# adamjorr/kbbq-py

Measured on AMD Instinct MI355X. Metric: bases/sec recalibrated (2x150 bp), higher is better.
Workload: dtype u8

## Files before the change

### kbbq-py_amd/csrc/kbbq_hip.hip

```cpp
#include "kbbq_kernels.h"
#include "kbbq_kernels_v3.h"
#include "kbbq_k2_tile.h"
#include "kbbq_solve_kernels.h"
#include "kbbq_lut_kernels.h"
#include "kbbq_aligned_kernels.h"
#include "kbbq_layout_kernels.h"
#include "kbbq_apply_aligned.h"
#include "kbbq_kmer.h"
#include "../../include/kbbq_hip.h"
#include "host_threads.h"

#include <algorithm>
#include <climits>
#include <cstdint>
#include <cstdarg>
#include <cstdio>
#include <cstring>
#include <functional>
#include <string>
#include <thread>
#include <vector>

static thread_local std::string g_err;

static int fail(int code, const char* fmt, ...)
{
    char buf[512];
    va_list ap; va_start(ap, fmt); vsnprintf(buf, sizeof buf, fmt, ap); va_end(ap);
    g_err = buf;
    return code;
}

static bool env_is(const char* name, const char* value) { const char* v = getenv(name); return v && !strcmp(v, value); }

int kbbq_set_error_(int code, const char* msg) { g_err = msg ? msg : ""; return code; }

#define HIPCHK(expr)                                                                   \
    do {                                                                               \
        hipError_t e_ = (expr);                                                        \
        if (e_ != hipSuccess)                                                          \
            return fail(KBBQ_E_HIP, "%s failed: %s (%s:%d)", #expr, hipGetErrorString(e_), \
                        __FILE__, __LINE__);                                           \
    } while (0)

struct DevScratch { void* p = nullptr; size_t bytes = 0; };

struct kbbq_ctx {
    int device = 0;
    int cus = 0;
    int lds_bytes = 0;
    char name[128] = {0};
    hipStream_t own_stream = nullptr;
    hipStream_t stream = nullptr;
    u64* d_status = nullptr;
    int* d_stats = nullptr;
    DevScratch wgplan;
    DevScratch ops4;
    DevScratch tally;
    DevScratch rowlut;
    void* stage_host[2] = {nullptr, nullptr}; void* stage_dev[2] = {nullptr, nullptr}; size_t stage_bytes = 0;
    hipStream_t stage_stream = nullptr;
    hipStream_t stage_down_stream = nullptr;
    hipEvent_t stage_up[2] = {nullptr, nullptr}, stage_used[2] = {nullptr, nullptr}, stage_down[2] = {nullptr, nullptr};
    bool timing = false;
    std::vector<std::pair<hipEvent_t, hipEvent_t>> ev[2];
    double ms_acc[2] = {0.0, 0.0};
    int64_t launches[2] = {0, 0};
};

#define KBBQ_NSTATUS 8

constexpr size_t K2T_ROW_LUT_MAX = 52 << 10;
constexpr int K2V3_FRONTS = 8;
constexpr int K2T_XCD_TILES = 1;
constexpr int K2T_XCD = 8;
constexpr int K7_FRONTS = 8;
constexpr int TALLY_K4_SHARE = 8;
static const u64 ST_INIT[KBBQ_NSTATUS] = {~0ull, ~0ull, ~0ull, ~0ull, ~0ull, ~0ull, ~0ull, ~0ull};

enum K1Form { K1_ROWS, K1_ALIGNED, K1_ALIGNED_REF, K1_BANDS };
struct K1Variant { K1Form form; int dn, nib, kj; const void* kernel[2]; };
#define K1_SPLITS(K, ...) {(const void*)(K<false, __VA_ARGS__>), (const void*)(K<true, __VA_ARGS__>)}
static const K1Variant K1_VARIANTS[] = {
    {K1_ROWS, K1V3_DNREP, 0, 0, K1_SPLITS(k1v3_accumulate, K1V3_DNREP)},
    {K1_ROWS, 8, 0, 0, K1_SPLITS(k1v3_accumulate, 8)},
    {K1_ROWS, K1V3_DNREP, 1, 0, K1_SPLITS(k1v3_accumulate, K1V3_DNREP, true)},
    {K1_ROWS, 8, 1, 0, K1_SPLITS(k1v3_accumulate, 8, true)},
    {K1_ROWS, K1V3_DNREP, 1, 13, K1_SPLITS(k1v3_accumulate, K1V3_DNREP, true, 13)},
    {K1_ROWS, K1V3_DNREP, 1, 19, K1_SPLITS(k1v3_accumulate, K1V3_DNREP, true, 19)},
    {K1_ALIGNED, K1V3_DNREP, 0, 0, K1_SPLITS(k1v3_aligned, K1V3_DNREP)},
    {K1_ALIGNED, 8, 0, 0, K1_SPLITS(k1v3_aligned, 8)},
    {K1_ALIGNED_REF, K1V3_DNREP, 0, 0, K1_SPLITS(k1v3_aligned_ref, K1V3_DNREP)},
    {K1_ALIGNED_REF, 8, 0, 0, K1_SPLITS(k1v3_aligned_ref, 8)},
    {K1_BANDS, 0, 0, 0, K1_SPLITS(k1v3_bands, false)},
    {K1_BANDS, 0, 1, 0, K1_SPLITS(k1v3_bands, true)},
};
#undef K1_SPLITS

static const void* k1_kernel(K1Form form, bool split, int dn, int nib, int kj)
{
    for (const K1Variant& v : K1_VARIANTS)
        if (v.form == form && v.dn == dn && v.nib == nib && v.kj == kj) return v.kernel[split];
    return nullptr;
}

enum LdsKernel { LK_K1_PLAIN, LK_K1_PLAIN_SPLIT, LK_K2V3, LK_K2V3_NIB, LK_K2T, LK_K2T_NIB, LK_K2T_BANDS, LK_K2_LDS16, LK_K2_LDS8, LK_COUNT };
static const void* const LDS_KERNELS[LK_COUNT] = {
    (const void*)k1_accumulate<false>, (const void*)k1_accumulate<true>,
    (const void*)k2v3_apply<false>, (const void*)k2v3_apply<true>,
    (const void*)k2t_apply<false>, (const void*)k2t_apply<true>, (const void*)k2t_bands,
    (const void*)k2_apply<int16_t, true, true>, (const void*)k2_apply<int8_t, true, false>,
};

extern "C" {

int kbbq_abi_version(void) { return KBBQ_ABI_VERSION; }
const char* kbbq_last_error(void) { return g_err.c_str(); }

int kbbq_device_count(int* count)
{
    int n = 0;
    hipError_t e = hipGetDeviceCount(&n);
    if (e != hipSuccess) { *count = 0; return fail(KBBQ_E_HIP, "hipGetDeviceCount: %s", hipGetErrorString(e)); }
    *count = n;
    return KBBQ_OK;
}

int kbbq_bind_host_to_device(int device, int* numa_node, int* ncpus)
{
    char busid[64] = {0};
    HIPCHK(hipDeviceGetPCIBusId(busid, (int)sizeof busid, device));
    return kbbq_bind_host_to_pci(busid, numa_node, ncpus);
}

int kbbq_ctx_create(int device, kbbq_ctx** out)
{
    if (!out) return fail(KBBQ_E_ARG, "kbbq_ctx_create: out is NULL");
    *out = nullptr;
    const bool dbg = getenv("KBBQ_CTX_DBG") != nullptr;
    auto t_prev = std::chrono::steady_clock::now();
    auto lap = [&](const char* what) {
        if (!dbg) return;
        const auto t = std::chrono::steady_clock::now();
        fprintf(stderr, "[kbbq_ctx_create] %-28s %7.2f ms\n", what, std::chrono::duration<double, std::milli>(t - t_prev).count());
        t_prev = t;
    };
    HIPCHK(hipSetDevice(device));
    lap("hipSetDevice");
    hipDeviceProp_t prop;
    HIPCHK(hipGetDeviceProperties(&prop, device));
    lap("hipGetDeviceProperties");
    if (strncmp(prop.gcnArchName, "gfx950", 6) != 0)
        return fail(KBBQ_E_HIP, "libkbbq_hip is built for gfx950 only; device %d is %s", device, prop.gcnArchName);
    kbbq_ctx* c = new kbbq_ctx();
    c->device = device;
    c->cus = prop.multiProcessorCount;
    c->lds_bytes = (int)prop.maxSharedMemoryPerMultiProcessor;
    if (c->lds_bytes <= 0) c->lds_bytes = 160 * 1024;
    snprintf(c->name, sizeof c->name, "%s (%s)", prop.name, prop.gcnArchName);
    hipError_t e = hipStreamCreateWithFlags(&c->own_stream, hipStreamNonBlocking);
    if (e != hipSuccess) { delete c; return fail(KBBQ_E_HIP, "hipStreamCreate: %s", hipGetErrorString(e)); }
    c->stream = c->own_stream;
    lap("hipStreamCreate");
    e = hipMalloc((void**)&c->d_status, sizeof ST_INIT);
    if (e != hipSuccess) { (void)hipStreamDestroy(c->own_stream); delete c; return fail(KBBQ_E_HIP, "hipMalloc(status): %s", hipGetErrorString(e)); }
    e = hipMemcpy(c->d_status, ST_INIT, sizeof ST_INIT, hipMemcpyHostToDevice);
    if (e != hipSuccess) { (void)hipFree(c->d_status); (void)hipStreamDestroy(c->own_stream); delete c; return fail(KBBQ_E_HIP, "hipMemcpy(status): %s", hipGetErrorString(e)); }
    lap("hipMalloc + hipMemcpy");
    auto full_lds = [&](const void* kernel) {
        (void)hipFuncSetAttribute(kernel, hipFuncAttributeMaxDynamicSharedMemorySize, c->lds_bytes);
        if (kernel == LDS_KERNELS[0]) lap("first hipFuncSetAttribute");
    };
    for (const void* kernel : LDS_KERNELS) full_lds(kernel);
    for (const K1Variant& v : K1_VARIANTS) { full_lds(v.kernel[0]); full_lds(v.kernel[1]); }
    (void)hipGetLastError();
    lap("the other attributes");
    *out = c;
    return KBBQ_OK;
}

int kbbq_ctx_destroy(kbbq_ctx* c)
{
    if (!c) return KBBQ_OK;
    (void)hipSetDevice(c->device);
    for (int w = 0; w < 2; ++w)
        for (auto& pr : c->ev[w]) { (void)hipEventDestroy(pr.first); (void)hipEventDestroy(pr.second); }
    if (c->d_status) (void)hipFree(c->d_status);
    if (c->d_stats) (void)hipFree(c->d_stats);
    for (DevScratch* s : {&c->wgplan, &c->ops4, &c->tally, &c->rowlut})
        if (s->p) (void)hipFree(s->p);
    for (int b = 0; b < 2; ++b) {
        if (c->stage_host[b]) (void)hipHostFree(c->stage_host[b]);
        if (c->stage_dev[b]) (void)hipFree(c->stage_dev[b]);
        if (c->stage_up[b]) (void)hipEventDestroy(c->stage_up[b]);
        if (c->stage_used[b]) (void)hipEventDestroy(c->stage_used[b]);
        if (c->stage_down[b]) (void)hipEventDestroy(c->stage_down[b]);
    }
    if (c->stage_stream) (void)hipStreamDestroy(c->stage_stream);
    if (c->stage_down_stream) (void)hipStreamDestroy(c->stage_down_stream);
    if (c->own_stream) (void)hipStreamDestroy(c->own_stream);
    delete c;
    return KBBQ_OK;
}

int kbbq_ctx_set_stream(kbbq_ctx* c, void* s)
{
    if (!c) return fail(KBBQ_E_ARG, "ctx is NULL");
    c->stream = (hipStream_t)s;
    return KBBQ_OK;
}

void* kbbq_ctx_stream_(kbbq_ctx* c) { return c ? (void*)c->stream : nullptr; }
int kbbq_ctx_device_(kbbq_ctx* c) { return c ? c->device : 0; }

int kbbq_ctx_sync(kbbq_ctx* c)
{
    if (!c) return fail(KBBQ_E_ARG, "ctx is NULL");
    HIPCHK(hipSetDevice(c->device));
    HIPCHK(hipStreamSynchronize(c->stream));
    return KBBQ_OK;
}

int kbbq_ctx_info(kbbq_ctx* c, int* cus, int* lds, char* name, int name_len)
{
    if (!c) return fail(KBBQ_E_ARG, "ctx is NULL");
    if (cus) *cus = c->cus;
    if (lds) *lds = c->lds_bytes;
    if (name && name_len > 0) { strncpy(name, c->name, (size_t)name_len - 1); name[name_len - 1] = 0; }
    return KBBQ_OK;
}

int kbbq_ctx_status(kbbq_ctx* c, int64_t* read_index)
{
    if (!c) return fail(KBBQ_E_ARG, "ctx is NULL");
    HIPCHK(hipSetDevice(c->device));
    u64 st[KBBQ_NSTATUS];
    HIPCHK(hipMemcpyAsync(st, c->d_status, sizeof st, hipMemcpyDeviceToHost, c->stream));
    HIPCHK(hipStreamSynchronize(c->stream));
    if (read_index) *read_index = -1;
    if (st[0] == ~0ull && st[1] == ~0ull && st[2] == ~0ull && st[3] == ~0ull && st[ST_MEANQ] == ~0ull && st[ST_KMER] == ~0ull)
        return KBBQ_OK;
    HIPCHK(hipMemcpyAsync(c->d_status, ST_INIT, sizeof ST_INIT, hipMemcpyHostToDevice, c->stream));
    HIPCHK(hipStreamSynchronize(c->stream));
    if (st[ST_KMER] != ~0ull)
        return fail(KBBQ_E_FULL, "k-mer table full: an insert found no free slot within %d probes (give the table more slots)",
                    KM_MAX_PROBES);
    if (st[0] == ~0ull && st[1] == ~0ull && st[2] == ~0ull && st[ST_MEANQ] != ~0ull) {
        if (read_index) *read_index = (int64_t)st[ST_MEANQ];
        return fail(KBBQ_E_MEANQ, "read group %lld: meanq lies on a truncation boundary (or the group has no counted base): "
                    "solve through kbbq_solve_dev with the host's longdouble meanq", (long long)st[ST_MEANQ]);
    }
    if (st[0] == ~0ull && st[1] == ~0ull && st[2] == ~0ull)
        return fail(KBBQ_E_LUT, "the device-built LUT can leave 0..255 or does not fit int8: re-run kbbq_apply_dev in checked mode");
    int code = KBBQ_E_TYPE; u64 best = st[ST_TYPE];
    if (st[ST_INDEX] < best) { best = st[ST_INDEX]; code = KBBQ_E_INDEX; }
    if (st[ST_RANGE] < best) { best = st[ST_RANGE]; code = KBBQ_E_RANGE; }
    if (read_index) *read_index = (int64_t)best;
    const char* what = code == KBBQ_E_TYPE ? "base outside ACGTN in a dinucleotide (reference: TypeError)"
                     : code == KBBQ_E_INDEX ? "quality/read-group/cycle beyond the tables (reference: IndexError)"
                                            : "recalibrated quality + 33 outside 0..255";
    return fail(code, "read %lld: %s", (long long)best, what);
}

// ... 699 lines not shown
                           int dinuc_minscore, const int64_t* d_seg, int64_t* d_tables, bool* fits, int S_band, int S_min, int nib, int twins,
                           K1Setup* setup_only)
{
    if (fits) *fits = true;
    if (S_band < 0 || S_band > S2 / 2 || (pairs && S_band)) return fail(KBBQ_E_ARG, "%s: S_band out of range (%d)", who, S_band);
    if (S_min < 0 || S_min > (S_band ? S_band : S2 / 2)) return fail(KBBQ_E_ARG, "%s: S_min out of range (%d)", who, S_min);
    int rc = check_planes(who, nrows, pitch, d_seq, d_cseq, d_qual);
    if (rc) return rc;
    if (R <= 0 || R > 32767) return fail(KBBQ_E_ARG, "%s: R out of range (%d)", who, R);
    if (S2 <= 0 || (S2 & 1) || S2 > 65534) return fail(KBBQ_E_ARG, "%s: S2 must be positive and even (%d)", who, S2);
    if (minscore < 0 || minscore > KQ - 1) return fail(KBBQ_E_ARG, "%s: minscore out of range (%d)", who, minscore);
    if (dinuc_minscore < 0 || dinuc_minscore > 222) return fail(KBBQ_E_ARG, "%s: dinuc_minscore out of range (%d)", who, dinuc_minscore);
    if (pairs && pitch != pair_pitch(S2)) return fail(KBBQ_E_ARG, "%s: mate-pair rows of %d-base reads have pitch %d, not %d", who, S2 / 2, pair_pitch(S2), pitch);
    if (nrows == 0) return KBBQ_OK;
    HIPCHK(hipSetDevice(c->device));
    const int S = S_band ? S_band : S2 / 2;
    K1Setup su;
    K1v3Params& q = su.q;
    q.aflags = nullptr; q.aclip = nullptr; q.atrim = nullptr;
    q.seq = d_seq; q.cseq = d_cseq; q.qual = d_qual; q.meta = d_meta;
    q.nreads = nrows; q.pitch = pitch; q.cpr = pitch / 16; q.cpr_magic = magic_for(q.cpr);
    q.R = R; q.S = S; q.gS2 = S2; q.minscore = minscore; q.type_minscore = dinuc_minscore;
    q.qlo_m1 = 32u + (u32)minscore; q.dlo = 33u + (u32)dinuc_minscore;
    q.nrows = KQ + 1 - minscore;
    q.maxlen = pairs ? S2 + 1 : S; q.gap = pairs ? 1 : 0; q.twins = (pairs && twins) ? 1 : 0;
    q.seg = reinterpret_cast<const long long*>(d_seg);
    q.tables = reinterpret_cast<u64*>(d_tables); q.status = c->d_status;
    q.genome = nullptr; q.ag0 = nullptr;
    const int trim = (!pairs && S_min > 0) ? std::min(S_min, S) : 0;
    if (pairs && nib && (q.cpr == 19 || q.cpr == 13)) {
        q.row_bytes = (u32)(((16 * q.cpr + 31) & ~31) * 4);
        q.minlen = 0; q.slack_bytes = 0; q.pos_copies = 1;
        q.dn_flush_iters = std::max(1, 65535 / ((K1V3_THREADS / K1V3_DNREP) * 16 * q.cpr));
        for (int nt = q.cpr == 19 ? 1 : 8; nt >= 1 && !su.dn; nt >>= 1) {
            const size_t rows = (size_t)q.nrows - 1 + nt;
            su.lds = rows * 128 * K1V3_DNREP + rows * q.row_bytes;
            if (su.lds > (size_t)c->lds_bytes) continue;
            su.dn = K1V3_DNREP; su.kj = q.cpr;
            q.ntrash = nt; q.pos_copy_bytes = (u32)(rows * q.row_bytes);
        }
    }
    for (int attempt = 0; attempt < (trim ? 3 : 1) && !su.dn; ++attempt) {
        const int copies = attempt == 2 ? 8 : K1V3_DNREP, cut = attempt ? trim : 0;
        if (k1_geometry(q, c, copies, cut, cut)) su.dn = copies;
    }
    if (!su.dn) {
        if (fits) { *fits = false; return KBBQ_OK; }
        return fail(KBBQ_E_LUT, "%s: %d-base reads with minscore %d do not fit the LDS tables; use plain one-read-per-row planes", who, S, minscore);
    }
    if (!su.kj) su.lds = k1_lds_plan(q, su.dn, c);
    if (setup_only) { *setup_only = su; return KBBQ_OK; }
    return launch_k1(c, K1_ROWS, su, nib);
}

int kbbq_accumulate_pairs_dev(kbbq_ctx* c, const uint8_t* d_pseq, const uint8_t* d_pcseq, const uint8_t* d_pqual,
                              const uint32_t* d_pmeta, int64_t npairs, int R, int S2, int minscore,
                              int dinuc_minscore, int64_t* d_tables)
{
    if (!c) return fail(KBBQ_E_ARG, "ctx is NULL");
    int rc = check_pairs("kbbq_accumulate_pairs_dev", npairs, S2);
    if (rc) return rc;
    return accumulate_rows(c, "kbbq_accumulate_pairs_dev", d_pseq, d_pcseq, d_pqual, d_pmeta, npairs, pair_pitch(S2), 1,
                           R, S2, minscore, dinuc_minscore, nullptr, d_tables, nullptr);
}

int kbbq_accumulate_grouped_dev(kbbq_ctx* c, const uint8_t* d_seq, const uint8_t* d_cseq, const uint8_t* d_qual,
                                const uint32_t* d_meta, int64_t nrows, int pitch, int pairs, int R, int S2, int S_band,
                                int S_min, int minscore, int dinuc_minscore, const int64_t* d_seg, int64_t* d_tables)
{
    if (!c) return fail(KBBQ_E_ARG, "ctx is NULL");
    if (!d_seg) return fail(KBBQ_E_ARG, "kbbq_accumulate_grouped_dev: d_seg is NULL");
    return accumulate_rows(c, "kbbq_accumulate_grouped_dev", d_seq, d_cseq, d_qual, d_meta, nrows, pitch, pairs ? 1 : 0,
                           R, S2, minscore, dinuc_minscore, d_seg, d_tables, nullptr, S_band, S_min);
}

int kbbq_pair_lut_dev(kbbq_ctx* c, const void* d_lut_blob, int R, int S2, int minscore, void* d_pair_lut)
{
    return kbbq_pair_lut_rows_dev(c, d_lut_blob, R, S2, minscore, KBBQ_ROWS_PAIRS, d_pair_lut);
}

int kbbq_pair_lut_rows_dev(kbbq_ctx* c, const void* d_lut_blob, int R, int S2, int minscore, int flags, void* d_pair_lut)
{
    if (!c) return fail(KBBQ_E_ARG, "ctx is NULL");
    int rc = check_pairs("kbbq_pair_lut_dev", 0, S2);
    if (rc) return rc;
    if (!(flags & KBBQ_ROWS_PAIRS) || (flags & ~(KBBQ_ROWS_PAIRS | KBBQ_ROWS_NIBBLES | KBBQ_ROWS_TWINS)))
        return fail(KBBQ_E_ARG, "kbbq_pair_lut_rows_dev: flags 0x%x are not those of mate-pair rows", flags);
    if (R <= 0 || R > 32767 || !d_lut_blob || !d_pair_lut) return fail(KBBQ_E_ARG, "kbbq_pair_lut_dev: bad argument");
    HIPCHK(hipSetDevice(c->device));
    PairLutParams f;
    f.lut16 = reinterpret_cast<const int16_t*>(d_lut_blob); f.rs16 = lut_row_stride(S2); f.R = R; f.Qt = KQ; f.S2 = S2;
    f.minscore = std::min(std::max(minscore, 0), KQ);
    f.twins = (flags & KBBQ_ROWS_TWINS) ? 1 : 0;
    f.out = reinterpret_cast<int8_t*>(d_pair_lut);
    hipLaunchKernelGGL(k3_fill_pair_lut, dim3((unsigned)(R * (33 + KQ))), dim3(256), 0, c->stream, f);
    HIPCHK(hipGetLastError());
    return KBBQ_OK;
}

static K2tParams k2t_params(const K2v3Params& q)
{
    K2tParams t;
    t.seq = q.seq; t.qual = q.qual; t.meta = q.meta; t.nchunks = q.nreads * q.cpr; t.cpr = q.cpr; t.cpr_magic = q.cpr_magic;
    t.Qt = q.Qt; t.S2 = q.S2; t.maxlen = q.maxlen; t.lut = q.full; t.lut_bytes = (int)(((size_t)(33 + q.Qt) * q.rb + 15) & ~(size_t)15);
    t.rb = q.rb; t.ctx_off = q.ctx_off; t.W = q.W; t.seg = q.seg; t.R = q.R; t.wg_start = nullptr; t.order = nullptr;
    t.perm = q.perm; t.pitch = q.pitch; t.out = q.out; t.status = q.status;
    t.xcd_tiles = K2T_XCD_TILES;
    return t;
}

static int apply_rows(kbbq_ctx* c, const char* who, const uint8_t* d_seq, const uint8_t* d_qual, const uint32_t* d_meta,
                      int64_t nrows, int pitch, int pairs, int R, int S2, int minscore, const void* d_lut_blob,
                      const void* d_pair_lut, const int64_t* d_seg, uint8_t* d_out, int nib, const int64_t* d_perm)
{
    int rc = check_planes(who, nrows, pitch, d_seq, d_qual, d_out);
    if (rc) return rc;
    if (R <= 0 || R > 32767 || !d_lut_blob || (pairs && (!d_pair_lut || ((uintptr_t)d_pair_lut & 15)))) return fail(KBBQ_E_ARG, "%s: bad argument", who);
    if (S2 <= 0 || (S2 & 1) || S2 > 65534) return fail(KBBQ_E_ARG, "%s: S2 must be positive and even (%d)", who, S2);
    if (minscore < 0 || minscore > 222) return fail(KBBQ_E_ARG, "%s: minscore out of range", who);
    if (pairs && pitch != pair_pitch(S2)) return fail(KBBQ_E_ARG, "%s: mate-pair rows of %d-base reads have pitch %d, not %d", who, S2 / 2, pair_pitch(S2), pitch);
    const int Sb = pairs ? S2 : row_lut_width(pitch, S2);
    K2v3Params q = k2v3_params(c, d_seq, d_qual, d_meta, nrows, pitch, pairs, R, KQ, S2, Sb, minscore, d_lut_blob, d_pair_lut, d_seg, d_perm, d_out);
    const size_t rg_bytes = (size_t)(33 + KQ) * q.rb;
    const size_t lds = d_seg ? rg_bytes : rg_bytes * (size_t)R;
    if (lds > (size_t)c->lds_bytes)
        return fail(KBBQ_E_LUT, "%s: the apply LUT (%zu B) does not fit the LDS; group the rows by read group or use kbbq_apply_dev", who, lds);
    if (nrows == 0) return KBBQ_OK;
    HIPCHK(hipSetDevice(c->device));
    if (!pairs && !narrowed_row_lut(c, d_lut_blob, R, KQ, S2, Sb, minscore, &q.full)) return fail(KBBQ_E_HIP, "%s: no scratch for the narrowed LUT", who);
    if (!k2_tile_serves(c, pairs, nib, R, d_seg != nullptr, q.cpr, rg_bytes)) return launch_k2v3(c, q, nib);

    K2tParams t = k2t_params(q);
    const int64_t per_wg = (int64_t)(K2T_THREADS / 64) * 64 * K2T_STEPS;
    int64_t gt = (t.nchunks + per_wg - 1) / per_wg;
    if (d_seg) {
        gt += R;
        const bool interleave = d_perm && R > 1;
        const int64_t ints = (int64_t)(R + 1) + 1 + (interleave ? 2 * gt : 0);
        if (ints > 0x7FFFFFFF) return fail(KBBQ_E_ARG, "%s: too many workgroups", who);
        rc = grow_scratch(c, c->wgplan, (size_t)ints * sizeof(int));
        if (rc) return rc;
        int* wg_start = reinterpret_cast<int*>(c->wgplan.p);
        K2tPlanParams pl; pl.seg = t.seg; pl.R = R; pl.cpr = q.cpr; pl.wg_start = wg_start;
        hipLaunchKernelGGL(k2t_plan, dim3(1), dim3(64), 0, c->stream, pl);
        t.wg_start = wg_start;
        if (interleave) {
            K2tOrderParams op; op.wg_start = wg_start; op.R = R;
            op.xcd = K2T_XCD;
            op.order = reinterpret_cast<int2*>(wg_start + ((R + 2) & ~1));
            hipLaunchKernelGGL(k2t_order, dim3((unsigned)((gt + 255) / 256)), dim3(256), 0, c->stream, op);
            t.order = op.order;
        }
    }
    return launch_lds(c, 1, LDS_KERNELS[nib ? LK_K2T_NIB : LK_K2T], dim3((unsigned)gt), dim3(K2T_THREADS), (size_t)t.lut_bytes, &t);
}

int kbbq_apply_pairs_dev(kbbq_ctx* c, const uint8_t* d_pseq, const uint8_t* d_pqual, const uint32_t* d_pmeta,
                         int64_t npairs, int R, int S2, int minscore, const void* d_lut_blob, const void* d_pair_lut,
                         uint8_t* d_pout)
{
    if (!c) return fail(KBBQ_E_ARG, "ctx is NULL");
    int rc = check_pairs("kbbq_apply_pairs_dev", npairs, S2);
    if (rc) return rc;
    return apply_rows(c, "kbbq_apply_pairs_dev", d_pseq, d_pqual, d_pmeta, npairs, pair_pitch(S2), 1, R, S2, minscore,
                      d_lut_blob, d_pair_lut, nullptr, d_pout);
}

int kbbq_apply_grouped_dev(kbbq_ctx* c, const uint8_t* d_seq, const uint8_t* d_qual, const uint32_t* d_meta,
                           int64_t nrows, int pitch, int pairs, int R, int S2, int minscore, const void* d_lut_blob,
                           const void* d_pair_lut, const int64_t* d_seg, uint8_t* d_out)
{
    if (!c) return fail(KBBQ_E_ARG, "ctx is NULL");
    if (!d_seg) return fail(KBBQ_E_ARG, "kbbq_apply_grouped_dev: d_seg is NULL");
    return apply_rows(c, "kbbq_apply_grouped_dev", d_seq, d_qual, d_meta, nrows, pitch, pairs ? 1 : 0, R, S2, minscore,
                      d_lut_blob, d_pair_lut, d_seg, d_out);
}


static int layout_flags_ok(const char* who, int flags)
{
    if (flags & ~(KBBQ_ROWS_PAIRS | KBBQ_ROWS_NIBBLES | KBBQ_ROWS_TWINS)) return fail(KBBQ_E_ARG, "%s: unknown layout flags 0x%x", who, flags);
    if ((flags & KBBQ_ROWS_TWINS) && !(flags & KBBQ_ROWS_PAIRS)) return fail(KBBQ_E_ARG, "%s: KBBQ_ROWS_TWINS describes mate-pair rows (add KBBQ_ROWS_PAIRS)", who);
    return KBBQ_OK;
}

int kbbq_accumulate_rows_dev(kbbq_ctx* c, const uint8_t* d_seq, const uint8_t* d_cseq, const uint8_t* d_qual,
                             const uint32_t* d_meta, int64_t nrows, int pitch, int flags, int R, int S2, int S_band,
                             int S_min, int minscore, int dinuc_minscore, const int64_t* d_seg, int64_t* d_tables)
{
    if (!c) return fail(KBBQ_E_ARG, "ctx is NULL");
    int rc = layout_flags_ok("kbbq_accumulate_rows_dev", flags);
    if (rc) return rc;
    const int pairs = (flags & KBBQ_ROWS_PAIRS) ? 1 : 0;
    if (pairs) { rc = check_pairs("kbbq_accumulate_rows_dev", nrows, S2); if (rc) return rc; }
    return accumulate_rows(c, "kbbq_accumulate_rows_dev", d_seq, d_cseq, d_qual, d_meta, nrows, pitch, pairs, R, S2, minscore,
                           dinuc_minscore, d_seg, d_tables, nullptr, pairs ? 0 : S_band, pairs ? 0 : S_min,
                           (flags & KBBQ_ROWS_NIBBLES) ? 1 : 0, (flags & KBBQ_ROWS_TWINS) ? 1 : 0);
}

int kbbq_apply_rows_dev(kbbq_ctx* c, const uint8_t* d_seq, const uint8_t* d_qual, const uint32_t* d_meta, int64_t nrows,
                        int pitch, int flags, int R, int S2, int minscore, const void* d_lut_blob, const void* d_pair_lut,
                        const int64_t* d_seg, const int64_t* d_perm, uint8_t* d_out)
{
    if (!c) return fail(KBBQ_E_ARG, "ctx is NULL");
    int rc = layout_flags_ok("kbbq_apply_rows_dev", flags);
    if (rc) return rc;
    const int pairs = (flags & KBBQ_ROWS_PAIRS) ? 1 : 0;
    if (pairs) { rc = check_pairs("kbbq_apply_rows_dev", nrows, S2); if (rc) return rc; }
    return apply_rows(c, "kbbq_apply_rows_dev", d_seq, d_qual, d_meta, nrows, pitch, pairs, R, S2, minscore, d_lut_blob,
                      d_pair_lut, d_seg, d_out, (flags & KBBQ_ROWS_NIBBLES) ? 1 : 0, d_perm);
}

static int band_accumulate_alone(kbbq_ctx* c, const kbbq_band& b, int R, int S2, int minscore, int dinuc_minscore, int64_t* d_tables)
{
    if (b.flags || b.d_seg)
        return kbbq_accumulate_rows_dev(c, b.d_seq, b.d_cseq, b.d_qual, b.d_meta, b.nrows, b.pitch, b.flags, R, S2, b.S_band, b.S_min,
                                        minscore, dinuc_minscore, b.d_seg, d_tables);
    return kbbq_accumulate_band_dev(c, b.d_seq, b.d_cseq, b.d_qual, b.d_meta, b.nrows, b.pitch, R, S2, b.S_band, b.S_min, minscore,
                                    dinuc_minscore, d_tables);
}

static void share_workgroups(const std::vector<double>& weight, const std::vector<int64_t>& cap, int total, std::vector<int>& out)
{
    const size_t n = weight.size();
    out.assign(n, 1);
    int left = total - (int)n;
    double sum = 0; for (double w : weight) sum += w;
    for (int round = 0; round < 4 && left > 0 && sum > 0; ++round) {
        std::vector<std::pair<double, size_t>> frac;
        int given = 0; double open_sum = 0;
        for (size_t i = 0; i < n; ++i) if (out[i] < cap[i]) open_sum += weight[i];
        if (open_sum <= 0) break;
        const int pool = left;
        for (size_t i = 0; i < n; ++i) {
            if (out[i] >= cap[i]) continue;
            const double want = pool * weight[i] / open_sum;
            int add = (int)std::min<int64_t>((int64_t)want, cap[i] - out[i]);
            out[i] += add; given += add;
            if (out[i] < cap[i]) frac.push_back({want - (int64_t)want, i});
        }
        left -= given;
        std::sort(frac.begin(), frac.end(), [](const auto& a, const auto& b) { return a.first > b.first; });
        for (auto& f : frac) { if (left <= 0) break; if (out[f.second] < cap[f.second]) { ++out[f.second]; --left; } }
    }
}

int kbbq_accumulate_bands_dev(kbbq_ctx* c, const kbbq_band* bands, int nbands, int R, int S2, int minscore, int dinuc_minscore,
                              int64_t* d_tables)
{
    if (!c) return fail(KBBQ_E_ARG, "ctx is NULL");
    if (nbands < 0 || (nbands > 0 && !bands)) return fail(KBBQ_E_ARG, "kbbq_accumulate_bands_dev: bad band list");
    std::vector<K1Setup> setups; std::vector<int> merged, alone;
    const bool merge = !env_is("KBBQ_K1_BANDS", "0");
    int nib_of_merge = -1;
    for (int i = 0; i < nbands; ++i) {
        const kbbq_band& b = bands[i];
        if (b.nrows == 0) continue;
        int rc = layout_flags_ok("kbbq_accumulate_bands_dev", b.flags);
        if (rc) return rc;
        const int pairs = (b.flags & KBBQ_ROWS_PAIRS) ? 1 : 0, nib = (b.flags & KBBQ_ROWS_NIBBLES) ? 1 : 0;
        K1Setup su; bool fits = false;
        bool can = merge && (int)merged.size() < K1V3_MAX_BANDS;
        if (can) {
            if (pairs) { rc = check_pairs("kbbq_accumulate_bands_dev", b.nrows, S2); if (rc) return rc; }
            rc = accumulate_rows(c, "kbbq_accumulate_bands_dev", b.d_seq, b.d_cseq, b.d_qual, b.d_meta, b.nrows, b.pitch, pairs, R, S2, minscore,
                                 dinuc_minscore, b.d_seg, d_tables, &fits, pairs ? 0 : b.S_band, pairs ? 0 : b.S_min, nib,
                                 (b.flags & KBBQ_ROWS_TWINS) ? 1 : 0, &su);
            if (rc) return rc;
            can = fits && !su.kj && (nib_of_merge < 0 || nib_of_merge == nib);
        }
        if (can) { nib_of_merge = nib; merged.push_back(i); setups.push_back(su); }
        else alone.push_back(i);
    }
    const int G = std::max(1, c->cus / std::max(R, 1));
    if (merged.size() < 2 || (int)merged.size() > G) { for (int i : merged) alone.push_back(i); merged.clear(); }
    for (int i : alone) {
        int rc = band_accumulate_alone(c, bands[i], R, S2, minscore, dinuc_minscore, d_tables);
        if (rc) return rc;
    }
    HIPCHK(hipSetDevice(c->device));
    if (merged.empty()) return KBBQ_OK;
    constexpr double row_cost = 1.25;
    constexpr double slope = 0.01;
    constexpr double dn8_cost = 1.06;
    K1BandsParams t;
    memset(&t, 0, sizeof t);
    t.nbands = (int)merged.size();
    std::vector<double> weight; std::vector<int64_t> cap; std::vector<int> share;
    size_t lds = 0;
    for (const K1Setup& su : setups) {
        weight.push_back((double)su.q.nreads * (su.q.cpr + row_cost) * (1.0 + slope * su.q.cpr) * (su.dn == K1V3_DNREP ? 1.0 : dn8_cost));
        cap.push_back(std::max<int64_t>(1, k1_iters(su.q)));
        lds = std::max(lds, su.lds);
    }
    share_workgroups(weight, cap, G, share);
    int run = 0;
    for (size_t j = 0; j < setups.size(); ++j) {
        t.wg_start[j] = run; run += share[j];
        t.dn[j] = setups[j].dn; t.band[j] = setups[j].q;
    }
    t.wg_start[setups.size()] = run;
    unsigned long long* dbg = nullptr;
    if (getenv("KBBQ_K1_BANDS_DBG")) { HIPCHK(hipMalloc((void**)&dbg, sizeof(unsigned long long) * 2 * (size_t)run)); t.dbg = dbg; }
    int rc = launch_lds(c, 0, k1_kernel(K1_BANDS, k1_split(setups[0].q), 0, nib_of_merge, 0), dim3((unsigned)run, (unsigned)R, 1),
                        dim3(K1V3_THREADS), lds, &t);
    if (rc) return rc;
    if (dbg) {
// ... 1377 lines not shown
```

### kbbq-py_amd/csrc/kbbq_k2_tile.h

```cpp
#pragma once
#include "kbbq_kernels_v3.h"

#define K2T_THREADS 1024
#define K2T_STEPS 4

struct K2tParams {
    const uint8_t* seq; const uint8_t* qual; const u32* meta;
    int xcd_tiles;
    long long nchunks;
    int cpr; u32 cpr_magic;
    int Qt; int S2; int maxlen;
    const int8_t* lut; int lut_bytes; u32 rb; u32 ctx_off;
    u32 W;
    const long long* seg;
    const int* wg_start;
    const int2* order;
    int R;
    const long long* perm;
    int pitch;
    uint8_t* out; u64* status;
};

struct K2tPlanParams { const long long* seg; int R; int cpr; int* wg_start; };
__global__ void k2t_plan(K2tPlanParams p)
{
    if (threadIdx.x != 0 || blockIdx.x != 0) return;
    const long long per = (long long)(K2T_THREADS / 64) * 64 * K2T_STEPS;
    long long run = 0;
    for (int g = 0; g < p.R; ++g) {
        p.wg_start[g] = (int)run;
        run += ((p.seg[g + 1] - p.seg[g]) * p.cpr + per - 1) / per;
    }
    p.wg_start[p.R] = (int)run;
}

struct K2tOrderParams { const int* wg_start; int R; int2* order; int xcd; };
__global__ __launch_bounds__(256) void k2t_order(K2tOrderParams p)
{
    const int b = (int)(blockIdx.x * blockDim.x + threadIdx.x);
    if (b >= p.wg_start[p.R]) return;
    int lo = 0, hi = p.R;
    while (hi - lo > 1) { const int mid = (lo + hi) >> 1; if (p.wg_start[mid] <= b) lo = mid; else hi = mid; }
    const int g = lo, i = b - p.wg_start[g];
    const long long ng = p.wg_start[g + 1] - p.wg_start[g];
    long long rank = 0;
    for (int h = 0; h < p.R; ++h) {
        const long long nh = p.wg_start[h + 1] - p.wg_start[h];
        if (nh == 0) continue;
        const long long A = (2ll * i + 1) * nh;
        const long long M = h < g ? A / ng : (A + ng - 1) / ng - 1;
        long long cnt = (M + 1) / 2;
        rank += cnt < nh ? cnt : nh;
    }
    if (p.xcd > 0) {
        const long long total = p.wg_start[p.R], win = (long long)p.xcd * p.R;
        const long long base = rank - rank % win;
        if (base + win <= total) { const long long r = rank - base; rank = base + r / p.R + (long long)p.xcd * (r % p.R); }
    }
    p.order[rank] = make_int2(g, i);
}

template <bool NIB>
__device__ __forceinline__ void k2t_body(const K2tParams& p, u32* lds, const int bx, const int ntiles)
{
    const int lane = lane_id();
    const int wave = __builtin_amdgcn_readfirstlane((int)(threadIdx.x >> 6));
    const int nwaves = K2T_THREADS / 64;
    int g = 0;
    long long chunk_lo = 0, chunk_hi = p.nchunks, wg = bx;
    long long tiles = ntiles;
    if (p.seg) {
        if (bx >= p.wg_start[p.R]) return;
        if (p.order) {
            const int2 o = p.order[bx];
            g = o.x; wg = o.y; tiles = 0;
        } else {
            int lo = 0, hi = p.R;
            while (hi - lo > 1) { const int mid = (lo + hi) >> 1; if (p.wg_start[mid] <= bx) lo = mid; else hi = mid; }
            g = lo;
            wg = (long long)bx - p.wg_start[g];
            tiles = p.wg_start[g + 1] - p.wg_start[g];
        }
        chunk_lo = p.seg[g] * p.cpr; chunk_hi = p.seg[g + 1] * p.cpr;
    }
    if (p.xcd_tiles) {
        const long long P = p.xcd_tiles == 1 ? 8 : p.xcd_tiles;
        tiles -= tiles % P;
        if (wg < tiles) wg = (wg % P) * (tiles / P) + wg / P;
    }
    const long long base = chunk_lo + (wg * nwaves + wave) * (64 * K2T_STEPS);
    const long long base_c = base < chunk_hi ? base : chunk_hi - 1;
    const long long row0 = base_c / p.cpr;
    const u32 rem0 = (u32)(base_c - row0 * p.cpr);
    u32 sq[K2T_STEPS][NIB ? 2 : 4], ql[K2T_STEPS][4], mk[K2T_STEPS];
    long long cidx[K2T_STEPS];
#pragma unroll
    for (int s = 0; s < K2T_STEPS; ++s) {
        const long long c = base + 64 * s + lane;
        const long long cc = c < chunk_hi ? c : chunk_hi - 1;
        cidx[s] = c;
        if constexpr (NIB) {
            const uint2 sv = *reinterpret_cast<const uint2*>(p.seq + 8 * cc);
            sq[s][0] = sv.x; sq[s][1] = sv.y;
        } else {
            const uint4 sv = *reinterpret_cast<const uint4*>(p.seq + 16 * cc);
            sq[s][0] = sv.x; sq[s][1] = sv.y; sq[s][2] = sv.z; sq[s][3] = sv.w;
        }
        const uint4 qv = *reinterpret_cast<const uint4*>(p.qual + 16 * cc);
        ql[s][0] = qv.x; ql[s][1] = qv.y; ql[s][2] = qv.z; ql[s][3] = qv.w;
        const u32 rel = rem0 + (u32)(cc - base_c);
        mk[s] = p.meta[row0 + __umulhi(rel, p.cpr_magic)];
    }
    const long long c0 = base < chunk_hi ? base : chunk_hi - 1;
    u32 before = 4u;
    if (c0 > 0) {
        if constexpr (NIB) before = (u32)p.seq[8 * c0 - 1] >> 4;
        else {
            u32 cd, cd5, expect;
            const u32 ch4 = (u32)p.seq[16 * c0 - 1] * 0x01010101u;
            decode4x(ch4, cd, cd5, expect);
            before = expect == ch4 ? (cd & 0xFFu) : 4u;
        }
    }
    {
        const uint4* src = reinterpret_cast<const uint4*>(p.lut + (size_t)g * (size_t)(33 + p.Qt) * p.rb);
        const int n16 = p.lut_bytes >> 4;
        for (int i = threadIdx.x; i < n16; i += K2T_THREADS) reinterpret_cast<uint4*>(lds)[i] = src[i];
        __syncthreads();
    }
    const u32 rb = p.rb;
    const u32 hi_add = (u32)(0x80 - (p.Qt + 33)) * 0x01010101u;
    u32 carry_code = 5u * before;
#pragma unroll
    for (int s = 0; s < K2T_STEPS; ++s) {
        const long long c = cidx[s];
        const bool act0 = c < chunk_hi;
        const u32 rel = rem0 + (u32)((act0 ? c : chunk_hi - 1) - base_c);
        const u32 drow = __umulhi(rel, p.cpr_magic);
        const long long row = row0 + drow;
        const int j = (int)(rel - drow * (u32)p.cpr);
        const int len = (int)(mk[s] & 0xFFFFu);
        const int nb = act0 ? len - 16 * j : 0;
        u32 code[4], code5[4], hiq = 0u, badbits = 0u;
        if constexpr (NIB) {
            code[0] = nib_lo(sq[s][0]); code[1] = nib_hi(sq[s][0]); code[2] = nib_lo(sq[s][1]); code[3] = nib_hi(sq[s][1]);
            badbits = nib_invalid(sq[s][0]) | nib_invalid(sq[s][1]);
        }
#pragma unroll
        for (int wd = 0; wd < 4; ++wd) {
            if constexpr (NIB) code5[wd] = (code[wd] << 2) + code[wd];
            else {
                u32 expect;
                decode4x(sq[s][wd], code[wd], code5[wd], expect);
                badbits |= expect ^ sq[s][wd];
            }
            hiq |= ((ql[s][wd] & 0x7F7F7F7Fu) + hi_add) | ql[s][wd];
        }
        hiq &= 0x80808080u;
        const u32 last_code5 = code5[3] >> 24;
        u32 prev_code5 = wave_shr1(last_code5, carry_code);
        carry_code = (u32)__builtin_amdgcn_readlane((int)last_code5, 63);
        if (j == 0) prev_code5 = 20u;
        if (act0) {
            u32 o[4] = {0u, 0u, 0u, 0u};
            if (nb > 0) {
                const int rg = (int)((mk[s] >> 16) & 0x7FFFu);
                if (hiq != 0u || rg != g || len > p.maxlen || badbits) {
                    flag(p.status, ST_LUT, 0);
                } else {
                    u32 d5[4];
                    u32 pc5 = prev_code5 << 24;
#pragma unroll
                    for (int wd = 0; wd < 4; ++wd) {
                        d5[wd] = __builtin_amdgcn_alignbyte(code5[wd], pc5, 3) + code[wd];
                        pc5 = code5[wd];
                    }
                    const u32 A = ((mk[s] >> 31) ? p.W : 0u) + (u32)(16 * j), C = p.ctx_off;
#pragma unroll
                    for (int wd = 0; wd < 4; ++wd) {
                        int v1[4], v2[4];
#pragma unroll
                        for (int b = 0; b < 4; ++b) {
                            const u32 qb = (ql[s][wd] >> (8 * b)) & 0xFFu;
                            const u32 rowq = __umul24(qb, rb);
                            const u32 dd = (d5[wd] >> (8 * b)) & 0xFFu;
                            v1[b] = *reinterpret_cast<const int8_t*>(reinterpret_cast<const char*>(lds) + (rowq + A + (u32)(4 * wd + b)));
                            v2[b] = *reinterpret_cast<const int8_t*>(reinterpret_cast<const char*>(lds) + (rowq + C + dd));
                        }
#pragma unroll
                        for (int b = 0; b < 4; ++b) o[wd] |= (u32)(v1[b] + v2[b] + 33) << (8 * b);
                    }
                }
            }
            uint8_t* dst = p.perm ? p.out + p.perm[row] * p.pitch + 16 * j : p.out + 16 * c;
            *reinterpret_cast<uint4*>(dst) = make_uint4(o[0], o[1], o[2], o[3]);
        }
    }
}

template <bool NIB = true>
__global__ __launch_bounds__(K2T_THREADS) void k2t_apply(K2tParams p)
{
    extern __shared__ __attribute__((aligned(16))) u32 lds[];
    k2t_body<NIB>(p, lds, (int)blockIdx.x, (int)gridDim.x);
}

#define K2T_MAX_BANDS 16
struct K2tBandsParams {
    int nbands;
    int wg_start[K2T_MAX_BANDS + 1];
    K2tParams band[K2T_MAX_BANDS];
};

__global__ __launch_bounds__(K2T_THREADS) void k2t_bands(K2tBandsParams t)
{
    extern __shared__ __attribute__((aligned(16))) u32 lds[];
    int lo = 0, hi = t.nbands;
    while (hi - lo > 1) { const int mid = (lo + hi) >> 1; if (t.wg_start[mid] <= (int)blockIdx.x) lo = mid; else hi = mid; }
    k2t_body<true>(t.band[lo], lds, (int)blockIdx.x - t.wg_start[lo], t.wg_start[lo + 1] - t.wg_start[lo]);
}
```

Baseline: 1132 billion.

## Add compile-time-geometry mate-pair apply kernel with SDWA byte-indexed LUT lookups

```diff
diff --git a/kbbq-py_amd/csrc/kbbq_hip.hip b/kbbq-py_amd/csrc/kbbq_hip.hip
--- a/kbbq-py_amd/csrc/kbbq_hip.hip
+++ b/kbbq-py_amd/csrc/kbbq_hip.hip
@@ -104,11 +104,12 @@
     return nullptr;
 }
 
-enum LdsKernel { LK_K1_PLAIN, LK_K1_PLAIN_SPLIT, LK_K2V3, LK_K2V3_NIB, LK_K2T, LK_K2T_NIB, LK_K2T_BANDS, LK_K2_LDS16, LK_K2_LDS8, LK_COUNT };
+enum LdsKernel { LK_K1_PLAIN, LK_K1_PLAIN_SPLIT, LK_K2V3, LK_K2V3_NIB, LK_K2T, LK_K2T_NIB, LK_K2T_BANDS, LK_K2T_PAIR19, LK_K2T_PAIR13, LK_K2_LDS16, LK_K2_LDS8, LK_COUNT };
 static const void* const LDS_KERNELS[LK_COUNT] = {
     (const void*)k1_accumulate<false>, (const void*)k1_accumulate<true>,
     (const void*)k2v3_apply<false>, (const void*)k2v3_apply<true>,
     (const void*)k2t_apply<false>, (const void*)k2t_apply<true>, (const void*)k2t_bands,
+    (const void*)k2t_apply_pair<19>, (const void*)k2t_apply_pair<13>,
     (const void*)k2_apply<int16_t, true, true>, (const void*)k2_apply<int8_t, true, false>,
 };
 
@@ -1114,7 +1115,10 @@
             t.order = op.order;
         }
     }
-    return launch_lds(c, 1, LDS_KERNELS[nib ? LK_K2T_NIB : LK_K2T], dim3((unsigned)gt), dim3(K2T_THREADS), (size_t)t.lut_bytes, &t);
+    const int kj = (pairs && nib) ? k2t_pair_form(t) : 0;
+    if (kj < 0) return fail(KBBQ_E_ARG, "%s: mate-pair rows of %d chunks do not have the geometry k2t_apply_pair was compiled for", who, q.cpr);
+    const LdsKernel k = kj == 19 ? LK_K2T_PAIR19 : kj == 13 ? LK_K2T_PAIR13 : nib ? LK_K2T_NIB : LK_K2T;
+    return launch_lds(c, 1, LDS_KERNELS[k], dim3((unsigned)gt), dim3(K2T_THREADS), (size_t)t.lut_bytes, &t);
 }
 
 int kbbq_apply_pairs_dev(kbbq_ctx* c, const uint8_t* d_pseq, const uint8_t* d_pqual, const uint32_t* d_pmeta,
diff --git a/kbbq-py_amd/csrc/kbbq_k2_tile.h b/kbbq-py_amd/csrc/kbbq_k2_tile.h
--- a/kbbq-py_amd/csrc/kbbq_k2_tile.h
+++ b/kbbq-py_amd/csrc/kbbq_k2_tile.h
@@ -1,5 +1,6 @@
 #pragma once
 #include "kbbq_kernels_v3.h"
+#include <type_traits>
 
 #define K2T_THREADS 1024
 #define K2T_STEPS 4
@@ -205,6 +206,176 @@
     k2t_body<NIB>(p, lds, (int)blockIdx.x, (int)gridDim.x);
 }
 
+template <int KJ> struct K2tPair {
+    static constexpr int PITCH = 16 * KJ;
+    static constexpr u32 CTX = (u32)PITCH;
+    static constexpr u32 RB = (u32)(PITCH + 32 + ((((PITCH + 32) >> 2) & 1) ? 0 : 4));
+    static constexpr u32 MAGIC = (u32)(((1ull << 32) + KJ - 1) / KJ);
+};
+
+template <int KJ> static inline bool k2t_pair_geometry(const K2tParams& t)
+{
+    return t.pitch == K2tPair<KJ>::PITCH && t.rb == K2tPair<KJ>::RB && t.ctx_off == K2tPair<KJ>::CTX && t.cpr_magic == K2tPair<KJ>::MAGIC
+           && t.W == 0u && t.xcd_tiles == 1 && t.rb == (u32)pair_lut_row_bytes(t.S2) && t.pitch == pair_pitch(t.S2);
+}
+static inline int k2t_pair_form(const K2tParams& t)
+{
+    if (t.cpr == 19) return k2t_pair_geometry<19>(t) ? 19 : -1;
+    if (t.cpr == 13) return k2t_pair_geometry<13>(t) ? 13 : -1;
+    return 0;
+}
+
+template <int B> __device__ __forceinline__ u32 k2t_mul24_byte(u32 w, u32 k)
+{
+    u32 r;
+    if constexpr (B == 0) asm("v_mul_u32_u24_sdwa %0, %1, %2 dst_sel:DWORD dst_unused:UNUSED_PAD src0_sel:BYTE_0 src1_sel:DWORD" : "=v"(r) : "v"(w), "v"(k));
+    else if constexpr (B == 1) asm("v_mul_u32_u24_sdwa %0, %1, %2 dst_sel:DWORD dst_unused:UNUSED_PAD src0_sel:BYTE_1 src1_sel:DWORD" : "=v"(r) : "v"(w), "v"(k));
+    else if constexpr (B == 2) asm("v_mul_u32_u24_sdwa %0, %1, %2 dst_sel:DWORD dst_unused:UNUSED_PAD src0_sel:BYTE_2 src1_sel:DWORD" : "=v"(r) : "v"(w), "v"(k));
+    else asm("v_mul_u32_u24_sdwa %0, %1, %2 dst_sel:DWORD dst_unused:UNUSED_PAD src0_sel:BYTE_3 src1_sel:DWORD" : "=v"(r) : "v"(w), "v"(k));
+    return r;
+}
+template <int B> __device__ __forceinline__ u32 k2t_add_byte(u32 a, u32 w)
+{
+    u32 r;
+    if constexpr (B == 0) asm("v_add_u32_sdwa %0, %1, %2 dst_sel:DWORD dst_unused:UNUSED_PAD src0_sel:DWORD src1_sel:BYTE_0" : "=v"(r) : "v"(a), "v"(w));
+    else if constexpr (B == 1) asm("v_add_u32_sdwa %0, %1, %2 dst_sel:DWORD dst_unused:UNUSED_PAD src0_sel:DWORD src1_sel:BYTE_1" : "=v"(r) : "v"(a), "v"(w));
+    else if constexpr (B == 2) asm("v_add_u32_sdwa %0, %1, %2 dst_sel:DWORD dst_unused:UNUSED_PAD src0_sel:DWORD src1_sel:BYTE_2" : "=v"(r) : "v"(a), "v"(w));
+    else asm("v_add_u32_sdwa %0, %1, %2 dst_sel:DWORD dst_unused:UNUSED_PAD src0_sel:DWORD src1_sel:BYTE_3" : "=v"(r) : "v"(a), "v"(w));
+    return r;
+}
+template <class F> __device__ __forceinline__ void k2t_unroll4(F f)
+{
+    f(std::integral_constant<int, 0>()); f(std::integral_constant<int, 1>()); f(std::integral_constant<int, 2>()); f(std::integral_constant<int, 3>());
+}
+
+typedef unsigned short k2t_u16x2 __attribute__((ext_vector_type(2)));
+
+template <int KJ>
+__global__ __launch_bounds__(K2T_THREADS) void k2t_apply_pair(K2tParams p)
+{
+    extern __shared__ __attribute__((aligned(16))) u32 lds[];
+    typedef K2tPair<KJ> G;
+    const u32 lane = (u32)lane_id();
+    const u32 wave = (u32)__builtin_amdgcn_readfirstlane((int)(threadIdx.x >> 6));
+    const int bx = (int)blockIdx.x;
+    int g = 0;
+    long long row_lo = 0, chunk_hi = p.nchunks;
+    u32 wg = (u32)bx, tiles = gridDim.x;
+    if (p.seg) {
+        if (bx >= p.wg_start[p.R]) return;
+        if (p.order) {
+            const int2 o = p.order[bx];
+            g = o.x; wg = (u32)o.y; tiles = 0u;
+        } else {
+            int lo = 0, hi = p.R;
+            while (hi - lo > 1) { const int mid = (lo + hi) >> 1; if (p.wg_start[mid] <= bx) lo = mid; else hi = mid; }
+            g = lo;
+            wg = (u32)(bx - p.wg_start[g]);
+            tiles = (u32)(p.wg_start[g + 1] - p.wg_start[g]);
+        }
+        row_lo = p.seg[g]; chunk_hi = p.seg[g + 1] * KJ;
+    }
+    tiles &= ~7u;
+    if (wg < tiles) wg = (wg & 7u) * (tiles >> 3) + (wg >> 3);
+    const long long chunk_lo = row_lo * KJ;
+    const long long base = chunk_lo + ((long long)wg * (K2T_THREADS / 64) + wave) * (64 * K2T_STEPS);
+    const bool has = base < chunk_hi;
+    const long long base_c = has ? base : chunk_hi - 1;
+    const unsigned long long off0 = (unsigned long long)(base_c - chunk_lo);
+    const unsigned long long rowd = off0 / (unsigned)KJ;
+    const u32 rem0 = (u32)(off0 - rowd * (unsigned)KJ);
+    const long long last = chunk_hi - 1 - base_c;
+    const u32 limit = last < 64 * K2T_STEPS - 1 ? (u32)last : (u32)(64 * K2T_STEPS - 1);
+    const uint8_t* qbase = p.qual + 16 * base_c;
+    const uint8_t* sbase = p.seq + 8 * base_c;
+    const u32* mbase = p.meta + (row_lo + (long long)rowd);
+    u32 sq[K2T_STEPS][2], ql[K2T_STEPS][4], mk[K2T_STEPS], a16[K2T_STEPS];
+#pragma unroll
+    for (int s = 0; s < K2T_STEPS; ++s) {
+        const u32 d = (u32)(64 * s) + lane;
+        const u32 dc = d < limit ? d : limit;
+        const uint2 sv = *reinterpret_cast<const uint2*>(sbase + 8u * dc);
+        sq[s][0] = sv.x; sq[s][1] = sv.y;
+        const uint4 qv = *reinterpret_cast<const uint4*>(qbase + 16u * dc);
+        ql[s][0] = qv.x; ql[s][1] = qv.y; ql[s][2] = qv.z; ql[s][3] = qv.w;
+        const u32 rel = rem0 + dc;
+        const u32 drow = __umulhi(rel, G::MAGIC);
+        a16[s] = 16u * (rel - drow * (u32)KJ);
+        mk[s] = mbase[drow];
+    }
+    u32 before = 4u;
+    if (base_c > 0) before = (u32)sbase[-1] >> 4;
+    {
+        const uint4* src = reinterpret_cast<const uint4*>(p.lut + (size_t)g * (size_t)(33 + p.Qt) * p.rb);
+        const int n16 = p.lut_bytes >> 4;
+        for (int i = threadIdx.x; i < n16; i += K2T_THREADS) reinterpret_cast<uint4*>(lds)[i] = src[i];
+        __syncthreads();
+    }
+    const uint8_t* L = reinterpret_cast<const uint8_t*>(lds);
+    const u32 rbv = G::RB;
+    const u32 hi_add = (u32)(0x80 - (p.Qt + 33)) * 0x01010101u;
+    u32 carry_code = 5u * before;
+#pragma unroll
+    for (int s = 0; s < K2T_STEPS; ++s) {
+        const u32 d = (u32)(64 * s) + lane;
+        const bool act0 = has && d <= limit;
+        const int len = (int)(mk[s] & 0xFFFFu);
+        const int nb = act0 ? len - (int)a16[s] : 0;
+        u32 code[4], code5[4], hiq = 0u;
+        code[0] = nib_lo(sq[s][0]); code[1] = nib_hi(sq[s][0]); code[2] = nib_lo(sq[s][1]); code[3] = nib_hi(sq[s][1]);
+        const u32 badbits = nib_invalid(sq[s][0]) | nib_invalid(sq[s][1]);
+#pragma unroll
+        for (int wd = 0; wd < 4; ++wd) {
+            code5[wd] = (code[wd] << 2) + code[wd];
+            hiq |= ((ql[s][wd] & 0x7F7F7F7Fu) + hi_add) | ql[s][wd];
+        }
+        hiq &= 0x80808080u;
+        const u32 last_code5 = code5[3] >> 24;
+        u32 prev_code5 = wave_shr1(last_code5, carry_code);
+        carry_code = (u32)__builtin_amdgcn_readlane((int)last_code5, 63);
+        if (a16[s] == 0u) prev_code5 = 20u;
+        if (act0) {
+            u32 o[4] = {0u, 0u, 0u, 0u};
+            if (nb > 0) {
+                const int rg = (int)((mk[s] >> 16) & 0x7FFFu);
+                if (hiq != 0u || rg != g || len > p.maxlen || badbits) {
+                    flag(p.status, ST_LUT, 0);
+                } else {
+                    u32 d5[4];
+                    u32 pc5 = prev_code5 << 24;
+#pragma unroll
+                    for (int wd = 0; wd < 4; ++wd) {
+                        d5[wd] = __builtin_amdgcn_alignbyte(code5[wd], pc5, 3) + code[wd];
+                        pc5 = code5[wd];
+                    }
+                    k2t_u16x2 cy[8], cx[8];
+#pragma unroll
+                    for (int wd = 0; wd < 4; ++wd) {
+                        k2t_unroll4([&](auto bc) {
+                            constexpr int b = decltype(bc)::value;
+                            const u32 t = k2t_mul24_byte<b>(ql[s][wd], rbv);
+                            cy[2 * wd + (b >> 1)][b & 1] = L[t + a16[s] + (u32)(4 * wd + b)];
+                            cx[2 * wd + (b >> 1)][b & 1] = L[k2t_add_byte<b>(t, d5[wd]) + G::CTX];
+                        });
+                    }
+#pragma unroll
+                    for (int wd = 0; wd < 4; ++wd) {
+                        const u32 lo = __builtin_bit_cast(u32, cy[2 * wd]) + __builtin_bit_cast(u32, cx[2 * wd]) + 0x00210021u;
+                        const u32 hi = __builtin_bit_cast(u32, cy[2 * wd + 1]) + __builtin_bit_cast(u32, cx[2 * wd + 1]) + 0x00210021u;
+                        o[wd] = __builtin_amdgcn_perm(hi, lo, 0x06040200u);
+                    }
+                }
+            }
+            uint8_t* dst = p.out + 16 * (base_c + d);
+            if (p.perm) {
+                const u32 rel = rem0 + d;
+                dst = p.out + p.perm[row_lo + (long long)rowd + __umulhi(rel, G::MAGIC)] * G::PITCH + a16[s];
+            }
+            *reinterpret_cast<uint4*>(dst) = make_uint4(o[0], o[1], o[2], o[3]);
+        }
+    }
+}
+
 #define K2T_MAX_BANDS 16
 struct K2tBandsParams {
     int nbands;
```

After: 1166 billion, median of 6. 1.03x the previous value.
